# jyakaranda/A-LeGO-LOAM

Hardware: AMD Instinct MI355X
Metric: scans/sec (16x1800 LiDAR) full IP->LO->LM loop (higher is better)
Workload: dtype f32/f64

## Files before the change

### a-lego-loam_amd/csrc/alego_api.hip

```cpp
#include <hip/hip_runtime.h>

#include <cmath>
#include <cstdio>
#include <cstdlib>
#include <algorithm>
#include <cstring>
#include <mutex>
#include <string>
#include <vector>

#include "../../include/alego_mi355x.h"
#include "api_gate.h"
#include "dev_common.h"
#include "dev_mem.h"
#include "front_end.h"
#include "lm_ctx.h"
#include "lm_host.h"
#include "merge_math.h"
#include "nn_rules.h"
#include "thin_math.h"
#include "occ_math.h"
#include "loop_ctx.h"
#include "pgraph.h"
#include "prof.h"
// ... 246 lines not shown
  d.ip_scr = ip_screen_consts(d.sin_ax, d.cos_ax, d.sin_ay, d.cos_ay, d.tan_theta, d.tan_g_lo, d.tan_g_hi, d.opt_ip_screen);
  d.opt_ip_fused = env_int("ALEGO_IP_FUSED", 1) != 0;
  d.opt_ip_half = env_int("ALEGO_IP_HALF", 1) != 0;
  d.opt_cc_fused = env_int("ALEGO_CC_FUSED", 1) != 0;
  d.opt_cc_tile = env_int("ALEGO_CC_TILE", 1) != 0;
  d.opt_ip_band = env_int("ALEGO_IP_BAND", 1) != 0;
  d.opt_fe_pick1 = env_int("ALEGO_FE_PICK1", 0) != 0;
  d.opt_fe_fused = env_int("ALEGO_FE_FUSED", 1) != 0;
  d.opt_fe_cand = env_int("ALEGO_FE_CAND", 0);
  d.opt_fe_span = env_int("ALEGO_FE_SPAN", 0);
  d.opt_lo_box_lds = env_int("ALEGO_LO_BOX_LDS", 1 << 20);
  d.opt_lo_grid = env_int("ALEGO_LO_GRID", 1) != 0;
  d.opt_fo_spin = env_int("ALEGO_FE_SPIN", 0);
  d.opt_fo_pad8 = env_int("ALEGO_FE_PAD8", 0) != 0;
  d.opt_map_merge = env_int("ALEGO_MAP_MERGE", 1) != 0;
  d.opt_solve_full_eval = env_int("ALEGO_SOLVE_FULL_EVAL", 0) != 0;
  d.fcap[F_SHARP] = d.cap_sharp * d.NS; d.fcap[F_LSHARP] = d.cap_lsharp * d.NS; d.fcap[F_FLAT] = d.cap_flat * d.NS; d.fcap[F_LFLAT] = d.N;
  d.lo_qcap_surf = d.fcap[F_FLAT]; d.lo_qcap_corner = d.fcap[F_SHARP];
  d.lo_box_cap = (d.N + LO_CH - 1) / LO_CH + d.NS;
  const size_t B = n_slots, N = d.N, NS = d.NS;
  int rc = 0;
  rc |= dalloc(h, &d.in_pts, B * ring_len * d.Pcap, false);
  rc |= dalloc(h, &d.in_n, B * ring_len);
  rc |= dalloc(h, &d.owner, B * N); rc |= dalloc(h, &d.range_img, B * N); rc |= dalloc(h, &d.flag_img, B * N);
  rc |= dalloc(h, &d.parent, B * N); rc |= dalloc(h, &d.cc_size, B * N); rc |= dalloc(h, &d.cc_rows, B * N);
  rc |= dalloc(h, &d.label_img, B * N); rc |= dalloc(h, &d.cc_label, B * N);
  d.ipb_col = nullptr; d.ipb_off = nullptr;
  if (d.NS > 16 && d.NS <= 64) { rc |= dalloc(h, &d.ipb_col, B * ipb_col_n(d)); rc |= dalloc(h, &d.ipb_off, B * ipb_off_n(d)); }
  d.ipf_own = nullptr;
  if (d.NS <= 16 && d.N <= 65535 && (d.H & 1) == 0) rc |= dalloc(h, &d.ipf_own, B * (N / 2), false);
// ... 707 lines not shown
  else if (s == "ALEGO_FE_FUSED") d.opt_fe_fused = value != 0;
  else if (s == "ALEGO_FE_CAND") d.opt_fe_cand = value;
  else if (s == "ALEGO_FE_SPAN") d.opt_fe_span = value;
  else if (s == "ALEGO_LO_BOX_LDS") d.opt_lo_box_lds = value;
  else if (s == "ALEGO_LO_GRID") d.opt_lo_grid = value != 0;
  else if (s == "ALEGO_FE_SPIN") d.opt_fo_spin = value;
  else if (s == "ALEGO_SOLVE_FULL_EVAL") d.opt_solve_full_eval = value != 0;
  else if (s == "ALEGO_FE_PAD8") d.opt_fo_pad8 = value != 0;
  else if (s == "ALEGO_FE_ERR_CLEAR") {
    if (value < -1 || value >= d.n_slots) return ALEGO_ERR_ARG;
    HIP_TRY(h, hipDeviceSynchronize());
    if (value >= 0) HIP_TRY(h, hipMemset(scal_of(d, value) + SC_FE_ERR, 0, 4));
    else HIP_TRY(h, hipMemset2D(scal_of(d, 0) + SC_FE_ERR, scal_n() * sizeof(int), 0, 4, d.n_slots));
  }
  else if (s == "ALEGO_MAP_MERGE") { if (int r = lm_host_set_map_merge(h->lm, value != 0, &h->err)) return r; d.opt_map_merge = value != 0; }
  else if (s == "ALEGO_IP_FAST") d.ip_fast = h->ip_fast_capable & value;
  else if (s == "ALEGO_POKE_GUARD") { HIP_TRY(h, hipMemset(scal_of(d, d.n_slots) + value, 0xFF, 4)); }
  else if (s == "ALEGO_GV_SMALL_MAX") { WAIT_ALL(h); return lm_host_set_gv_small_max(h->lm, value); }
  else if (s == "ALEGO_LOC_CHUNK") return lm_host_set_loc_chunk(h->lm, value);
  else if (s == "ALEGO_PG_BUDGET") graph_ctx_set_budget(&h->pg, value);
  else if (s == "ALEGO_LC_BUDGET") loop_ctx_set_budget(&h->lc, value);
  else if (s == "ALEGO_RL_BUDGET") reloc_ctx_set(&h->rl, 0, value);
  else if (s == "ALEGO_RL_BRUTE") reloc_ctx_set(&h->rl, 1, value);
  else if (s == "ALEGO_SHARD_SLICE") return lm_host_debug_slice(h->lm, value & 0xff, value >> 8, &h->err);
  else { h->err = "unknown option " + s; return ALEGO_ERR_ARG; }
  return 0;
}

int alego_loop_detect(const alego_params* P, const float* keyposes6, const double* stamps, int32_t n, const double cur_xyz[3]) {
  if (!P || n <= 0 || !keyposes6 || !stamps || !cur_xyz) return -1;
// ... 834 lines not shown
```

### a-lego-loam_amd/csrc/dev_common.h

```cpp
#ifndef ALEGO_DEV_COMMON_H_
#define ALEGO_DEV_COMMON_H_

#include <hip/hip_runtime.h>
#include <stdint.h>

#include "../../include/alego_params.h"
#include "wave.h"
#include "ip_pred.h"

#define IPB_NM 9
#define IP_OWNER_TAG 0x40000000

struct DevCtx {
  alego_params P;
  int n_slots, ring_len;
  int slot0, n_launch;
  int N, H, NS;
  int Pcap;
  int cap_sharp, cap_lsharp, cap_flat;
  double sin_ax, cos_ax, sin_ay, cos_ay;
  double inv_res_x, inv_res_y;
  const double2* ip_rowtab;
  const double2* ip_coltab;
  const double* ip_colfrac;
// ... 1 lines not shown
  unsigned h_magic;
  double tan_g_lo, tan_g_hi;
  double tan_theta;
  IpScreenConsts ip_scr;
  int opt_ip_fused;
  int opt_ip_half;
  int opt_cc_fused;
  int opt_cc_tile;
  int opt_fe_pick1;
  int opt_fe_fused;
  int opt_fe_cand;
  int opt_fe_span;
  int opt_lo_box_lds;
  int opt_map_merge;
  int opt_ip_screen;
  int opt_solve_full_eval;
  float4* in_pts;
  int* in_n;
  const float4* bag_pts;
  const int* bag_n;
  const int2* bag_src;
  int n_bags, bag_len, replay_bag;
  int fs_cur, fs_last;
  int* owner;
  float* range_img;
  uint8_t* flag_img;
  int* parent;
  int* cc_size;
  unsigned long long* cc_rows;
  unsigned long long* ipb_col;
// ... 170 lines not shown
```

### a-lego-loam_amd/csrc/kernels_lm.hip

```cpp
#include <cstddef>
#include <cstring>

#include "../../include/alego_mi355x.h"
#include "dev_cost.h"
#include "nn_rules.h"
#include "remap_math.h"
#include "prof.h"
#include "kf_store.h"
#include "gmap.h"
#include "vgrid.h"

#define LM_BLOCK 256

DEV_INLINE double* ldp(const LmCtx& L, int slot) { return L.ld + (size_t)slot * LD_COUNT; }
DEV_INLINE int* lip(const LmCtx& L, int slot) { return L.li + (size_t)slot * LI_COUNT; }

DEV_INLINE void lm_map_update(const LmCtx& L, int slot, int* li, int merge) {
  const int nkf = li[LI_NKF];
  if (nkf == 0) return;
  int* rec = L.rec + (size_t)slot * L.K;
  const int cnt = li[LI_REC_CNT];
  bool changed = false;
  if (cnt < L.K) {
    const int nk = min(nkf, L.K);
    changed = li[LI_DIRTY] != 0;
// ... 101 lines not shown
  if (j == nk - 1 && blockIdx.x == 0 && threadIdx.x == 0) { li[LI_KRAW_C] = offc + nc; li[LI_KRAW_S] = offs + ns + no; }
}

__global__ void __launch_bounds__(LM_BLOCK) lm_total(DevCtx d, LmCtx L) {
  const int slot = blockIdx.y + d.slot0;
  int* li = lip(L, slot);
  if (!li[LI_RUN]) return;
  int ns = li[LI_NCUR_S], no = li[LI_NCUR_O];
  if (ns + no > L.total_cap) { no = L.total_cap - ns; if (threadIdx.x == 0 && blockIdx.x == 0) li[LI_OVERFLOW] = 1; }
  const float4* s = L.cur_surf_ds + (size_t)slot * L.kf_cap_s;
  const float4* o = L.cur_outl_ds + (size_t)slot * L.kf_cap_o;
  float4* t = L.cur_total + (size_t)slot * L.total_cap;
  for (int i = blockIdx.x * LM_BLOCK + threadIdx.x; i < ns; i += gridDim.x * LM_BLOCK) t[i] = s[i];
  for (int i = blockIdx.x * LM_BLOCK + threadIdx.x; i < no; i += gridDim.x * LM_BLOCK) t[ns + i] = o[i];
  if (blockIdx.x == 0 && threadIdx.x == 0) li[LI_NTOTAL] = ns + no;
}

DEV_INLINE int grid_cell(const GridGeom& g, float x, float y, float z, int* cx, int* cy, int* cz) {
  *cx = nn_lm_coord(x, g.inv) - g.ox; *cy = nn_lm_coord(y, g.inv) - g.oy; *cz = nn_lm_coord(z, g.inv) - g.oz;
  return nn_lm_index(*cx, *cy, *cz, g.gx, g.gy, g.gz);
}

__global__ void __launch_bounds__(LM_BLOCK) lm_grid_build(DevCtx d, LmCtx L) {
  const int slot = blockIdx.y + d.slot0, m = blockIdx.x;
  const int* li = lip(L, slot);
  if (!li[LI_REBUILD]) return;
  __shared__ GridGeom s_g;
  __shared__ int s[LM_BLOCK / 64];
  __shared__ int s_run;
  if (threadIdx.x == 0) {
// ... 921 lines not shown
void launch_lm_prepare(const DevCtx& d, const LmCtx& L, int stage, int run_hint, int par, hipStream_t st) {
  const bool small = run_hint == 0 || stage == 2;
  const dim3 grid = small ? dim3(1, 1, d.n_launch) : dim3(8, 3, d.n_launch);
  ALEGO_LAUNCH(lm_prepare, grid, dim3(small ? 64 : LM_BLOCK), 0, st, d, L, stage, run_hint, par);
}
void launch_lm_stage(const DevCtx& d, const LmCtx& L, int run_hint, int par, hipStream_t st) {
  const dim3 grid = run_hint == 0 ? dim3(1, 1, d.n_launch) : dim3(8, 3, d.n_launch);
  ALEGO_LAUNCH(lm_stage, grid, dim3(run_hint == 0 ? 64 : LM_BLOCK), 0, st, d, L, run_hint, par);
}
void launch_lm_concat(const DevCtx& d, const LmCtx& L, hipStream_t st) {
  ALEGO_LAUNCH(lm_concat, dim3(2, L.K, d.n_launch), dim3(LM_BLOCK), 0, st, d, L);
}
void launch_lm_total(const DevCtx& d, const LmCtx& L, hipStream_t st) {
  ALEGO_LAUNCH(lm_total, dim3(8, d.n_launch), dim3(LM_BLOCK), 0, st, d, L);
}
void launch_lm_grid(const DevCtx& d, const LmCtx& L, hipStream_t st) {
  ALEGO_LAUNCH(lm_grid_build, dim3(2, d.n_launch), dim3(LM_BLOCK), 0, st, d, L);
}
void launch_lm_solve(const DevCtx& d, const LmCtx& L, bool remap, hipStream_t st) {
  const size_t lds = LM_SOLVE_RED_BYTES + L.solve_row_bytes;
  if (remap) {
    if (d.opt_solve_full_eval) ALEGO_LAUNCH(lm_solve_remap_full_eval, dim3(d.n_launch), dim3(LM_SOLVE_T), lds, st, d, L);
    else ALEGO_LAUNCH(lm_solve_remap, dim3(d.n_launch), dim3(LM_SOLVE_T), lds, st, d, L);
  } else if (d.opt_solve_full_eval) {
    ALEGO_LAUNCH(lm_solve_full_eval, dim3(d.n_launch), dim3(LM_SOLVE_T), lds, st, d, L);
  } else {
    ALEGO_LAUNCH(lm_solve, dim3(d.n_launch), dim3(LM_SOLVE_T), lds, st, d, L);
  }
}
int launch_lm_register(const DevCtx& d, const LmCtx& L, hipStream_t st, int (*allreduce)(void*, double*, size_t, hipStream_t), void* ar_ctx) {
// ... 70 lines not shown
```

### a-lego-loam_amd/csrc/kernels_voxel.hip

```cpp
#include <algorithm>
#include <cstring>

#include <hip/hip_runtime.h>

#include <vector>

#include "voxel.h"
#include "wave.h"
#include "vgrid.h"
#include "dev_mem.h"
#include "prof.h"

typedef unsigned long long u64;

__device__ __forceinline__ bool vx_enabled(const VoxJob& J) { return J.enable == nullptr || *J.enable != 0; }

#ifndef VX_SMALL_MAX
#define VX_SMALL_MAX 8192
#endif

#ifndef VG_T
#define VG_T 512
#endif
#define VG_W (VG_T / 64)
#define VG_DMAX 9
#define VG_ND (1 << VG_DMAX)
#define VG_U 4

__device__ __forceinline__ int vg_div(int pos, int seglen, double inv_seglen) {
  int q = (int)((double)pos * inv_seglen);
  if (q * seglen > pos) --q;
  if ((q + 1) * seglen <= pos) ++q;
  return q;
}
// ... 385 lines not shown
    for (int j = blockIdx.x; j < nbig; j += min((int)gridDim.x, V.grid_big)) {
      vox_big_job(V, V.list_big[j], vs_smem_k);
      __syncthreads();
    }
  }
}

__global__ void __launch_bounds__(256) vox_plan(VoxCtx V) {
  __shared__ int s_n[2];
  if (threadIdx.x < 2) s_n[threadIdx.x] = 0;
  __syncthreads();
  for (int j = threadIdx.x; j < V.njobs; j += 256) {
    const VoxJob J = V.jobs[j];
    if (!vx_enabled(J)) continue;
    const int n = min(*J.n_in, J.cap);
    if (n == 0) { *J.n_out = 0; if (J.mode == 1 && J.n_sel_out) J.n_sel_out[(size_t)(J.out_sel ? *J.out_sel : 0) * J.n_sel_stride] = 0; continue; }
    if (n <= VX_SMALL_MAX) V.list_small[atomicAdd(&s_n[0], 1)] = j;
    else V.list_big[atomicAdd(&s_n[1], 1)] = j;
  }
  __syncthreads();
  if (threadIdx.x < 2) V.cnt[threadIdx.x] = s_n[threadIdx.x];
}

#define VX_SMALL_LDS (8 * VX_SMALL_MAX + 2 * VS_W * VS_ND)
int vox_create(VoxCtx* V, const VoxJob* jobs, int njobs, std::string* err) {
  std::memset(V, 0, sizeof(*V));
  if (hipFuncSetAttribute(reinterpret_cast<const void*>(vox_small), hipFuncAttributeMaxDynamicSharedMemorySize, VX_SMALL_LDS) != hipSuccess) { *err = "vox_create: hipFuncSetAttribute"; return -2; }
  std::vector<VoxJob> h(jobs, jobs + njobs);
  size_t total = 0;
  for (auto& j : h) {
    j.off = (int)total;
    if (j.cap > VX_SMALL_MAX) total += (size_t)j.cap;
  }
  if (total > 0x7fffffffull) { *err = "vox_create: scratch exceeds 2^31 elements"; return -3; }
  V->njobs = njobs; V->total = (unsigned)total;
  hipError_t e = hipSuccess;
  DevPool mem;
  auto A = [&](auto** p, size_t count) { if (e == hipSuccess) e = mem.get(p, count, true); };
  A(&V->jobs, (size_t)njobs); A(&V->bbox, (size_t)njobs * 8);
  A(&V->keys, total); A(&V->pairs_a, total); A(&V->pairs_b, total);
  A(&V->list_small, (size_t)njobs); A(&V->list_big, (size_t)njobs); A(&V->cnt, 2);
  V->grid_small = V->grid_big = njobs;
  if (e == hipSuccess) e = hipMemcpy(V->jobs, h.data(), sizeof(VoxJob) * njobs, hipMemcpyHostToDevice);
  if (e != hipSuccess) { std::memset(V, 0, sizeof(*V)); *err = std::string("vox_create: ") + hipGetErrorString(e); return -2; }
  mem.detach();
  return 0;
}

void vox_destroy(VoxCtx* V) {
  DevPool mem;
  for (void* p : {(void*)V->jobs, (void*)V->bbox, (void*)V->keys, (void*)V->pairs_a, (void*)V->pairs_b, (void*)V->list_small, (void*)V->list_big, (void*)V->cnt}) mem.adopt(p);
  std::memset(V, 0, sizeof(*V));
}

int vox_run(const VoxCtx& V, hipStream_t st, std::string* err) {
  (void)err;
  if (V.njobs == 0) return 0;
  ALEGO_LAUNCH(vox_plan, dim3(1), dim3(256), 0, st, V);
  static_assert(VG_T == VX_SB && VG_LDS_BYTES <= VX_SMALL_LDS, "large jobs run in vox_small's workgroups and LDS");
  ALEGO_LAUNCH(vox_small, dim3(std::max(V.grid_small, V.grid_big)), dim3(VX_SB), (size_t)VX_SMALL_LDS, st, V);
  return 0;
}
```

### a-lego-loam_amd/csrc/lm_ctx.h

```cpp
#ifndef ALEGO_LM_CTX_H_
#define ALEGO_LM_CTX_H_
#include "dev_common.h"
#include "lm_rows.h"

enum {
  LI_NKF = 0,
  LI_DIRTY,
  LI_RUN,
  LI_REBUILD,
  LI_FRAME,
  LI_FLAGS,
  LI_NCC, LI_NSC,
  LI_SUM0, LI_SUM1,
  LI_KF_ADDED, LI_OPTIMIZED,
  LI_KRAW_C, LI_KRAW_S, LI_KDS_C, LI_KDS_S,
  LI_NIN_C, LI_NIN_S, LI_NIN_O,
  LI_NCUR_C, LI_NCUR_S, LI_NCUR_O,
  LI_NTOTAL, LI_NTOTAL_DS,
  LI_NREBUILD,
  LI_OVERFLOW,
  LI_REC_CNT,
  LI_LATEST,
  LI_NU_C, LI_NU_S,
  LI_UVALID,
  LI_PREV_CNT,
  LI_KF_PENDING,
  LI_KF_PEND_RING,
  LI_TMPN_C, LI_TMPN_S,
  LI_REBUILD_FB,
  LI_MAP_PASS,
  LI_SORT_N,
  LI_SORT_N1,
  LI_COUNT = 48
};
enum {
  LD_PARAMS = 0,
  LD_T_M2O = 6, LD_Q_M2O = 9,
  LD_T_O2L = 13, LD_Q_O2L = 16,
  LD_T_M2L = 20, LD_Q_M2L = 23,
  LD_PARAMS_IT = 27,
  LD_COSTS = 39,
  LD_LOC_P = 44,
  LD_COUNT = 48
};

struct alego_graph_edge;
struct alego_regcov;
struct alego_remap;

struct MapWork {
  int* items;
  int* count;
  int cap;
};
struct GridGeom { int ox, oy, oz; float inv; int gx, gy, gz, ncell; };


DEV_INLINE void keypose_matrix(const float* kp, float m[3][4]) {
  const float hz = 0.5f * kp[5], hy = 0.5f * kp[4], hx = 0.5f * kp[3];
  const float qz[4] = {d_cosf(hz), 0.f, 0.f, d_sinf(hz)};
  const float qy[4] = {d_cosf(hy), 0.f, d_sinf(hy), 0.f};
  const float qx[4] = {d_cosf(hx), d_sinf(hx), 0.f, 0.f};
  float t[4], q[4];
  t[0] = qz[0] * qy[0] - qz[1] * qy[1] - qz[2] * qy[2] - qz[3] * qy[3];
  t[1] = qz[0] * qy[1] + qz[1] * qy[0] + qz[2] * qy[3] - qz[3] * qy[2];
  t[2] = qz[0] * qy[2] + qz[2] * qy[0] + qz[3] * qy[1] - qz[1] * qy[3];
  t[3] = qz[0] * qy[3] + qz[3] * qy[0] + qz[1] * qy[2] - qz[2] * qy[1];
  q[0] = t[0] * qx[0] - t[1] * qx[1] - t[2] * qx[2] - t[3] * qx[3];
  q[1] = t[0] * qx[1] + t[1] * qx[0] + t[2] * qx[3] - t[3] * qx[2];
// ... 100 lines not shown
  }
}
DEV_INLINE void lm_store_outer_empty(int* li, double* ld, int outer) {
  if (outer < 2) {
    li[LI_SUM0 + outer] = 4 << 16;
    for (int k = 0; k < 6; ++k) ld[LD_PARAMS_IT + outer * 6 + k] = ld[LD_PARAMS + k];
  }
}

size_t lm_solve_row_bytes_max(), lm_solve_row_bytes_default();
int lm_configure();
void launch_lm_prepare(const DevCtx& d, const LmCtx& L, int stage, int run_hint, int par, hipStream_t st);
void launch_lm_stage(const DevCtx& d, const LmCtx& L, int run_hint, int par, hipStream_t st);
void launch_lm_concat(const DevCtx& d, const LmCtx& L, hipStream_t st);
void launch_lm_total(const DevCtx& d, const LmCtx& L, hipStream_t st);
void launch_lm_grid(const DevCtx& d, const LmCtx& L, hipStream_t st);
void launch_lm_solve(const DevCtx& d, const LmCtx& L, bool remap, hipStream_t st);
int launch_lm_register(const DevCtx& d, const LmCtx& L, hipStream_t st, int (*allreduce)(void*, double*, size_t, hipStream_t), void* ar_ctx);
void launch_lm_retransform(const DevCtx& d, const LmCtx& L, int ring, hipStream_t st);
void launch_lm_apply_correction(const DevCtx& d, const LmCtx& L, int slot, const double* rc_dev, hipStream_t st);
void launch_lm_regcov_debug(const double* blocks, const float4* qc, int n_edge, const float4* qs, int n_plane, const double* params, double huber, const double* opt,
                            alego_regcov* rec, hipStream_t st);
void regcov_host(const double* acc28, const double* params6, int n_edge, int n_plane, const double* opt, alego_regcov* out);
void regcov_normal_host(const double* params6, const double* edge_rows9, int n_edge, const double* plane_rows7, int n_plane, double huber, double* acc28);
void remap_host(const double* acc28, const double* params6, int n_edge, int n_plane, double eig_min, alego_remap* out);
int remap_step_host(const double* H21, const double* g6, const double* scale6, double radius, const double* proj36, double* step6, double* mcc);
void launch_map_update(const DevCtx& d, const LmCtx& L, const MapWork& W, hipStream_t st);
void launch_map_accum(const DevCtx& d, const LmCtx& L, const MapWork& W, hipStream_t st);
void launch_loc_select(const DevCtx& d, const LmCtx& L, hipStream_t st);

// ... 2 lines not shown
```

### a-lego-loam_amd/csrc/lm_host.hip

```cpp
#include "lm_host.h"
#include "api_gate.h"
#include "dev_mem.h"

#include <cstddef>
#include <cstdio>
#include <cstdlib>
#include <algorithm>
#include <cstring>
#include <vector>

#include <rccl/rccl.h>

#include "kf_store.h"
#include "voxel.h"
#include "gmap.h"
#include "loc_math.h"
#include "pgraph.h"
#include "merge.h"
#include "merge_math.h"
#include "thin.h"
#include "thin_math.h"
#include "occ.h"
#include "loc_store.h"
#include "remap_math.h"

struct LmHost {
  alego_params P;
  int n_slots;
  int gsize;
  std::vector<hipStream_t> st;
  LmCtx L;
  std::vector<VoxCtx> vm, v2;
  std::vector<VoxCtx> vk;
  std::vector<MapWork> work;
  bool fallback_ok = true;
  ncclComm_t comm = nullptr;
  std::string dist_err;
  DevPool mem;
  std::vector<long> frames;
  GvCtx gv;
  int* arc_off = nullptr;
  VoxCtx vloc;
  bool vloc_made = false;
  int loc_chunk = 128;
  DevBuf<MgPair> mg_pairs;
  DevBuf<int2> mg_items;
  DevBuf<int> mg_tail;
  DevBuf<MgMove> mg_moves;
  DevBuf<ThJob> th_jobs;
// ... 111 lines not shown
  if (hipMemcpy(L.ld, ld.data(), ld.size() * sizeof(double), hipMemcpyHostToDevice) != hipSuccess) { *err = "lm_host_create: upload failed"; lm_host_destroy(lm); return nullptr; }
  std::vector<int> li0(B * LI_COUNT, 0);
  for (size_t b = 0; b < B; ++b) li0[b * LI_COUNT + LI_LATEST] = -1;
  if (hipMemcpy(L.li, li0.data(), li0.size() * sizeof(int), hipMemcpyHostToDevice) != hipSuccess) { *err = "lm_host_create: upload failed"; lm_host_destroy(lm); return nullptr; }
  for (size_t g = 0; g < st.size(); ++g) {
  std::vector<VoxJob> jm, j1, j2, jk;
  for (size_t b = g * gsize; b < B && b < (g + 1) * (size_t)gsize; ++b) {
    int* li = L.li + b * LI_COUNT;
    if (lm->fallback_ok) {
      jm.push_back(VoxJob{L.map_corner_raw + b * L.map_cap_c, li + LI_KRAW_C, L.map_corner_ds + b * L.map_cap_c, li + LI_KDS_C, li + LI_REBUILD_FB, P.lm_leaf_corner, L.map_cap_c, L.map_cap_c, li + LI_OVERFLOW, 0});
      jm.push_back(VoxJob{L.map_surf_raw + b * L.map_cap_s, li + LI_KRAW_S, L.map_surf_ds + b * L.map_cap_s, li + LI_KDS_S, li + LI_REBUILD_FB, P.lm_leaf_surf, L.map_cap_s, L.map_cap_s, li + LI_OVERFLOW, 0});
    }
    j1.push_back(VoxJob{L.in_corner + b * L.in_cap_c, li + LI_NIN_C, L.cur_corner_ds + b * L.kf_cap_c, li + LI_NCUR_C, li + LI_RUN, P.lm_leaf_corner, L.in_cap_c, L.kf_cap_c, li + LI_OVERFLOW, 0});
    j1.push_back(VoxJob{L.in_surf + b * L.in_cap_s, li + LI_NIN_S, L.cur_surf_ds + b * L.kf_cap_s, li + LI_NCUR_S, li + LI_RUN, P.lm_leaf_surf, L.in_cap_s, L.kf_cap_s, li + LI_OVERFLOW, 0});
    j1.push_back(VoxJob{L.in_outl + b * L.in_cap_o, li + LI_NIN_O, L.cur_outl_ds + b * L.kf_cap_o, li + LI_NCUR_O, li + LI_RUN, P.lm_leaf_outlier, L.in_cap_o, L.kf_cap_o, li + LI_OVERFLOW, 0});
    j2.push_back(VoxJob{L.cur_total + b * L.total_cap, li + LI_NTOTAL, L.cur_total_ds + b * L.total_cap, li + LI_NTOTAL_DS, li + LI_RUN, P.lm_leaf_surf, L.total_cap, L.total_cap, li + LI_OVERFLOW, 0});
    kf_sort_jobs(L, P, (int)b, &jk);
  }
  const int ns = (int)j1.size() / 3;
  jm.insert(jm.end(), j1.begin(), j1.end());
  jm.insert(jm.end(), jk.begin(), jk.end());
  if (vox_create(&lm->vm[g], jm.data(), (int)jm.size(), err) || vox_create(&lm->v2[g], j2.data(), (int)j2.size(), err) ||
      vox_create(&lm->vk[g], jk.data(), (int)jk.size(), err)) { lm_host_destroy(lm); return nullptr; }
  const bool big_scans = d.N > 8 * 8192;
  lm->vm[g].grid_small = 3 * ns + std::max(2, ns / 2);
  if (const char* e = getenv("ALEGO_VOX_GRID_DIV")) { const int dv = std::max(1, atoi(e)); lm->vm[g].grid_small = std::max(2, lm->vm[g].grid_small / dv); lm->v2[g].grid_small = std::max(1, lm->v2[g].grid_small / dv); }
  lm->vm[g].grid_big = (!d.opt_map_merge || big_scans) ? std::max(2, ns / 2) : std::min(8, std::max(2, ns / 2));
  lm->v2[g].grid_big = big_scans ? std::max(2, ns / 2) : std::max(1, ns / 16);
  lm->vk[g].grid_small = 2; lm->vk[g].grid_big = 2;
  MapWork& W = lm->work[g];
  W.cap = std::max(4096, 64 * ns);
  if (!A(lm, &W.items, (size_t)W.cap, err) || !A(lm, &W.count, 2, err)) { lm_host_destroy(lm); return nullptr; }
  }
  return lm;
}

void lm_host_destroy(LmHost* lm) {
  if (!lm) return;
  if (lm->comm) { (void)ncclCommDestroy(lm->comm); lm->comm = nullptr; }
  for (auto& v : lm->vm) vox_destroy(&v);
  for (auto& v : lm->v2) vox_destroy(&v);
  for (auto& v : lm->vk) vox_destroy(&v);
  if (lm->vloc_made) vox_destroy(&lm->vloc);
  gv_destroy(&lm->gv);
// ... 7 lines not shown
  static const bool on = getenv("ALEGO_DEBUG_SYNC") != nullptr;
  if (!on) return true;
  hipError_t e = hipStreamSynchronize(st);
  if (e == hipSuccess) e = hipGetLastError();
  fprintf(stderr, "[alego dbg] %s: %s\n", what, hipGetErrorString(e));
  if (e != hipSuccess) { *err = std::string(what) + ": " + hipGetErrorString(e); return false; }
  return true;
}

static int map_sequence(LmHost* lm, const DevCtx& d, const LmCtx& L, int g, hipStream_t st, std::string* err) {
  if (!d.opt_map_merge) {
    if (!lm->fallback_ok) { *err = "ALEGO_MAP_MERGE=0 needs the handle to be created with it (more than 64 slots)"; return ALEGO_ERR_ARG; }
    launch_lm_concat(d, L, st);
    if (!dbg_sync(st, "lm_concat", err)) return ALEGO_ERR_HIP;
  }
  if (int r = vox_run(lm->vm[g], st, err)) return r;
  if (!dbg_sync(st, "vox round 1", err)) return ALEGO_ERR_HIP;
  launch_map_update(d, L, lm->work[g], st);
  if (!dbg_sync(st, "map_update", err)) return ALEGO_ERR_HIP;
  if (d.opt_map_merge) {
    launch_map_accum(d, L, lm->work[g], st);
    if (!dbg_sync(st, "map_accum", err)) return ALEGO_ERR_HIP;
  }
  launch_lm_grid(d, L, st);
  if (!dbg_sync(st, "lm_grid", err)) return ALEGO_ERR_HIP;
  return 0;
}

static int lm_allreduce(void* ctx, double* buf, size_t count, hipStream_t st) {
  LmHost* lm = static_cast<LmHost*>(ctx);
  const ncclResult_t r = ncclAllReduce(buf, buf, count, ncclDouble, ncclSum, lm->comm, st);
// ... 20 lines not shown
    par = (int)(A->k & 1);
    if (A->k >= 2 && hipStreamWaitEvent(A->front, A->back_same, 0) != hipSuccess) { *err = "hipStreamWaitEvent failed"; return ALEGO_ERR_HIP; }
    if (hint != 0 && A->k >= 1 && hipStreamWaitEvent(A->front, A->back_other, 0) != hipSuccess) { *err = "hipStreamWaitEvent failed"; return ALEGO_ERR_HIP; }
    launch_lm_stage(d, L, hint, par, A->front);
    if (hipEventRecord(A->staged, A->front) != hipSuccess || hipStreamWaitEvent(st, A->staged, 0) != hipSuccess) { *err = "event hand-over to the LaserMapping stream failed"; return ALEGO_ERR_HIP; }
    stage = 2;
  }
  launch_lm_prepare(d, L, stage, hint, par, st);
  if (!dbg_sync(st, "lm_prepare", err)) return ALEGO_ERR_HIP;
  if (n_run == 0) return 0;
  if (L.loc_on) {
    launch_loc_select(d, L, st);
    if (!dbg_sync(st, "loc_select", err)) return ALEGO_ERR_HIP;
  }
  if (int r = map_sequence(lm, d, L, g, st, err)) return r;
  launch_lm_total(d, L, st);
  if (int r = vox_run(lm->v2[g], st, err)) return r;
  if (!dbg_sync(st, "vox total", err)) return ALEGO_ERR_HIP;
  if (int r = launch_lm_register(d, L, st, lm->comm ? &lm_allreduce : nullptr, lm)) { *err = "sharded registration: " + lm->dist_err; return r; }
  if (!dbg_sync(st, "lm_register", err)) return ALEGO_ERR_HIP;
  return 0;
}

static void clear_run_flags_outside(LmHost* lm, const DevCtx& d) {
  const int g = d.slot0 / lm->gsize;
  const int lo = g * lm->gsize, hi = std::min(lm->n_slots, lo + lm->gsize);
  if (d.slot0 == lo && d.slot0 + d.n_launch == hi) return;
  for (int s = lo; s < hi; ++s) {
    if (s >= d.slot0 && s < d.slot0 + d.n_launch) continue;
    (void)hipMemsetAsync(lm->L.li + (size_t)s * LI_COUNT + LI_RUN, 0, sizeof(int), lm->st[g]);
  }
}
// ... 1136 lines not shown
```

### a-lego-loam_amd/csrc/vgrid.h

```cpp
#ifndef ALEGO_VGRID_H_
#define ALEGO_VGRID_H_
#include <hip/hip_runtime.h>

__device__ __forceinline__ unsigned vgr_enc(float f) {
  const unsigned b = (unsigned)__float_as_int(f);
  return b ^ ((b >> 31) ? 0xFFFFFFFFu : 0x80000000u);
}
__device__ __forceinline__ float vgr_dec(unsigned u) { return __int_as_float((int)((u >> 31) ? (u ^ 0x80000000u) : ~u)); }
__device__ __forceinline__ void vgr_box_load(const unsigned* bb, float mn[3], float mx[3]) {
#pragma unroll
  for (int a = 0; a < 3; ++a) { mn[a] = vgr_dec(bb[a]); mx[a] = vgr_dec(~bb[4 + a]); }
}

__device__ __forceinline__ void vgr_box_add(float mn[3], float mx[3], float4 p) {
  mn[0] = fminf(mn[0], p.x); mn[1] = fminf(mn[1], p.y); mn[2] = fminf(mn[2], p.z);
  mx[0] = fmaxf(mx[0], p.x); mx[1] = fmaxf(mx[1], p.y); mx[2] = fmaxf(mx[2], p.z);
}

__device__ __forceinline__ bool vgr_leaf_too_small(const float mn[3], const float mx[3], float inv) {
  const long long dx = (long long)((mx[0] - mn[0]) * inv) + 1, dy = (long long)((mx[1] - mn[1]) * inv) + 1, dz = (long long)((mx[2] - mn[2]) * inv) + 1;
  return dx * dy * dz > 2147483647LL;
}

struct VgrGeom {
  int minb[3], divb[3];
  unsigned mul1, mul2;
  unsigned long long T;
};
__device__ __forceinline__ VgrGeom vgr_geom(const float mn[3], const float mx[3], float inv) {
  VgrGeom g;
#pragma unroll
  for (int a = 0; a < 3; ++a) { g.minb[a] = (int)floorf(mn[a] * inv); g.divb[a] = (int)floorf(mx[a] * inv) - g.minb[a] + 1; }
  g.mul1 = (unsigned)g.divb[0];
  g.mul2 = (unsigned)g.divb[0] * (unsigned)g.divb[1];
  g.T = (unsigned long long)(unsigned)g.divb[0] * (unsigned)g.divb[1] * (unsigned)g.divb[2];
  return g;
}
__device__ __forceinline__ int vgr_bits(unsigned long long T) {
  if (T > 0xFFFFFFFFull || T == 0) return 32;
  return T > 1 ? 32 - __clz((int)(unsigned)(T - 1)) : 0;
}
__device__ __forceinline__ void vgr_coords(const VgrGeom& g, float4 p, float inv, int* i0, int* i1, int* i2) {
  *i0 = (int)(floorf(p.x * inv) - (float)g.minb[0]);
  *i1 = (int)(floorf(p.y * inv) - (float)g.minb[1]);
  *i2 = (int)(floorf(p.z * inv) - (float)g.minb[2]);
}
__device__ __forceinline__ unsigned vgr_id(const VgrGeom& g, float4 p, float inv) {
  int i0, i1, i2;
  vgr_coords(g, p, inv, &i0, &i1, &i2);
  return (unsigned)i0 + (unsigned)i1 * g.mul1 + (unsigned)i2 * g.mul2;
}

#define VKEY_B (1 << 20)
__device__ __forceinline__ bool vkey_holds_box(const float mn[3], const float mx[3], float inv) {
#pragma unroll
  for (int a = 0; a < 3; ++a)
    if (floorf(mn[a] * inv) < -(float)VKEY_B || floorf(mx[a] * inv) > (float)(VKEY_B - 1)) return false;
  return true;
}
__device__ __forceinline__ unsigned long long vkey_pack(int ix, int iy, int iz) {
  const int B = VKEY_B;
  const unsigned long long x = (unsigned long long)(unsigned)min(max(ix + B, 0), 2 * B - 1), y = (unsigned long long)(unsigned)min(max(iy + B, 0), 2 * B - 1),
                           z = (unsigned long long)(unsigned)min(max(iz + B, 0), 2 * B - 1);
  return (z << 42) | (y << 21) | x;
}
__device__ __forceinline__ unsigned long long vkey_of(const float4& p, float inv) {
  return vkey_pack((int)floorf(p.x * inv), (int)floorf(p.y * inv), (int)floorf(p.z * inv));
}

#endif
```

### a-lego-loam_amd/csrc/voxel.h

```cpp
#ifndef ALEGO_VOXEL_H_
#define ALEGO_VOXEL_H_
#include <hip/hip_runtime.h>

#include <string>

struct VoxJob {
  const float4* in;
  const int* n_in;
  float4* out;
  int* n_out;
  const int* enable;
  float leaf;
  int cap;
  int out_cap;
  int* overflow;
  int off;
  int mode;
  const int* out_sel;
  int out_stride;
  float* box_out;
  int* n_sel_out;
  int n_sel_stride;
};

struct VoxCtx {
  VoxJob* jobs;
  int njobs;
  unsigned* bbox;
  unsigned* keys;
  unsigned long long *pairs_a, *pairs_b;
  int *list_small, *list_big, *cnt;
  int grid_small, grid_big;
  unsigned total;
};

int vox_create(VoxCtx* V, const VoxJob* jobs, int njobs, std::string* err);
void vox_destroy(VoxCtx* V);
int vox_run(const VoxCtx& V, hipStream_t st, std::string* err);

#endif
```

Measured before the change: 490,900.

## Fuse outlier voxelization and surf/outlier total merge into one LM kernel

Adds a single-block-per-slot kernel that voxel-downsamples small outlier clouds in LDS and then merges the already-sorted surface voxels with the outlier voxels into the total downsampled cloud. Only slots whose merge cannot be proven sound fall back to the generic voxel path, through a device-built work list. This removes the separate outlier voxel job, the concat kernel and most of the generic total voxel pass. The cost is an O(n^2) rank sort in LDS, a dependence on the surface cloud being key-sorted (checked at runtime, with fallback), and extra code paths behind a default-on flag.

After: 498,600 (median of 6 runs). 1.6% higher.

```diff
diff --git a/a-lego-loam_amd/csrc/alego_api.hip b/a-lego-loam_amd/csrc/alego_api.hip
--- a/a-lego-loam_amd/csrc/alego_api.hip
+++ b/a-lego-loam_amd/csrc/alego_api.hip
@@ -284,6 +284,7 @@
   d.opt_fo_spin = env_int("ALEGO_FE_SPIN", 0);
   d.opt_fo_pad8 = env_int("ALEGO_FE_PAD8", 0) != 0;
   d.opt_map_merge = env_int("ALEGO_MAP_MERGE", 1) != 0;
+  d.opt_lm_total_merge = env_int("ALEGO_LM_TOTAL_MERGE", 1) != 0;
   d.opt_solve_full_eval = env_int("ALEGO_SOLVE_FULL_EVAL", 0) != 0;
   d.fcap[F_SHARP] = d.cap_sharp * d.NS; d.fcap[F_LSHARP] = d.cap_lsharp * d.NS; d.fcap[F_FLAT] = d.cap_flat * d.NS; d.fcap[F_LFLAT] = d.N;
   d.lo_qcap_surf = d.fcap[F_FLAT]; d.lo_qcap_corner = d.fcap[F_SHARP];
@@ -1021,6 +1022,7 @@
     else HIP_TRY(h, hipMemset2D(scal_of(d, 0) + SC_FE_ERR, scal_n() * sizeof(int), 0, 4, d.n_slots));
   }
   else if (s == "ALEGO_MAP_MERGE") { if (int r = lm_host_set_map_merge(h->lm, value != 0, &h->err)) return r; d.opt_map_merge = value != 0; }
+  else if (s == "ALEGO_LM_TOTAL_MERGE") d.opt_lm_total_merge = value != 0;
   else if (s == "ALEGO_IP_FAST") d.ip_fast = h->ip_fast_capable & value;
   else if (s == "ALEGO_POKE_GUARD") { HIP_TRY(h, hipMemset(scal_of(d, d.n_slots) + value, 0xFF, 4)); }
   else if (s == "ALEGO_GV_SMALL_MAX") { WAIT_ALL(h); return lm_host_set_gv_small_max(h->lm, value); }
diff --git a/a-lego-loam_amd/csrc/dev_common.h b/a-lego-loam_amd/csrc/dev_common.h
--- a/a-lego-loam_amd/csrc/dev_common.h
+++ b/a-lego-loam_amd/csrc/dev_common.h
@@ -39,6 +39,7 @@
   int opt_lo_box_lds;
   int opt_map_merge;
   int opt_ip_screen;
+  int opt_lm_total_merge;
   int opt_solve_full_eval;
   float4* in_pts;
   int* in_n;
diff --git a/a-lego-loam_amd/csrc/kernels_lm.hip b/a-lego-loam_amd/csrc/kernels_lm.hip
--- a/a-lego-loam_amd/csrc/kernels_lm.hip
+++ b/a-lego-loam_amd/csrc/kernels_lm.hip
@@ -9,6 +9,7 @@
 #include "kf_store.h"
 #include "gmap.h"
 #include "vgrid.h"
+#include "vox_merge.h"
 
 #define LM_BLOCK 256
 
@@ -140,6 +141,188 @@
   for (int i = blockIdx.x * LM_BLOCK + threadIdx.x; i < ns; i += gridDim.x * LM_BLOCK) t[i] = s[i];
   for (int i = blockIdx.x * LM_BLOCK + threadIdx.x; i < no; i += gridDim.x * LM_BLOCK) t[ns + i] = o[i];
   if (blockIdx.x == 0 && threadIdx.x == 0) li[LI_NTOTAL] = ns + no;
+}
+
+#define LT_T 256
+#define LT_B 8
+DEV_INLINE void lt_box_reduce(float mn[3], float mx[3], float (*s_red)[LT_T / 64]) {
+  const int lane = threadIdx.x & 63, wave = threadIdx.x >> 6;
+  __syncthreads();
+#pragma unroll
+  for (int a = 0; a < 3; ++a) {
+    bfly_minmax_f32(mn[a], mx[a]);
+    if (lane == 0) { s_red[a][wave] = mn[a]; s_red[3 + a][wave] = mx[a]; }
+  }
+  __syncthreads();
+#pragma unroll
+  for (int a = 0; a < 3; ++a) {
+    mn[a] = s_red[a][0]; mx[a] = s_red[3 + a][0];
+#pragma unroll
+    for (int w = 1; w < LT_T / 64; ++w) { mn[a] = fminf(mn[a], s_red[a][w]); mx[a] = fmaxf(mx[a], s_red[3 + a][w]); }
+  }
+}
+DEV_INLINE void lt_order(const vm_u64* s_key, vm_u64* s_skey, unsigned short* s_idx, int n) {
+  __syncthreads();
+  for (int i = threadIdx.x; i < n; i += LT_T) { const int r = vm_rank(s_key, n, i); s_skey[r] = s_key[i]; s_idx[r] = (unsigned short)i; }
+  __syncthreads();
+}
+
+__global__ void __launch_bounds__(LT_T) lm_total_merge(DevCtx d, LmCtx L, LtLists W) {
+  const int slot = blockIdx.x + d.slot0, tid = threadIdx.x;
+  int* li = lip(L, slot);
+  __shared__ vm_u64 s_key[LT_OCAP], s_skey[LT_OCAP];
+  __shared__ unsigned short s_idx[LT_OCAP];
+  __shared__ int s_osb[LT_OCAP];
+  __shared__ int s_oop[LT_OCAP + 1];
+  __shared__ int s_base[LT_T];
+  __shared__ float s_red[6][LT_T / 64];
+  __shared__ int s_w[LT_T / 64];
+  int state = 0;
+  if (li[LI_RUN]) {
+    const float FMAX = 3.402823466e+38f;
+    int no = li[LI_NCUR_O];
+    const int nin = min(li[LI_NIN_O], L.in_cap_o);
+    if (nin <= LT_OCAP) {
+      const float4* in = L.in_outl + (size_t)slot * L.in_cap_o;
+      float4* out = L.cur_outl_ds + (size_t)slot * L.kf_cap_o;
+      const int cap = L.kf_cap_o;
+      const float inv = 1.0f / d.P.lm_leaf_outlier;
+      int nvox = 0, full = nin;
+      if (nin > 0) {
+        float mn[3] = {FMAX, FMAX, FMAX}, mx[3] = {-FMAX, -FMAX, -FMAX};
+        for (int i = tid; i < nin; i += LT_T) vgr_box_add(mn, mx, in[i]);
+        lt_box_reduce(mn, mx, s_red);
+        if (vgr_leaf_too_small(mn, mx, inv)) {
+          for (int i = tid; i < min(nin, cap); i += LT_T) out[i] = in[i];
+        } else {
+          const VgrGeom g = vgr_geom(mn, mx, inv);
+          for (int i = tid; i < nin; i += LT_T) s_key[i] = vgr_id(g, in[i], inv);
+          lt_order(s_key, s_skey, s_idx, nin);
+          for (int t0 = 0; t0 < nin; t0 += LT_T) {
+            const int m = t0 + tid;
+            const bool head = m < nin && (m == 0 || s_skey[m] != s_skey[m - 1]);
+            int tot;
+            const int r = nvox + block_excl_scan<LT_T / 64>(head ? 1 : 0, s_w, &tot);
+            if (head && r < cap) {
+              int b = m + 1;
+              while (b < nin && s_skey[b] == s_skey[m]) ++b;
+              out[r] = vm_centroid([&](int j) { return in[s_idx[j]]; }, m, b);
+            }
+            nvox += tot;
+          }
+          full = nvox;
+        }
+      }
+      no = min(full, cap);
+      if (tid == 0) { li[LI_NCUR_O] = no; if (full > cap) li[LI_OVERFLOW] = 1; }
+      __syncthreads();
+    }
+    const int ns = li[LI_NCUR_S];
+    if (ns + no > L.total_cap) { no = L.total_cap - ns; if (tid == 0) li[LI_OVERFLOW] = 1; }
+    const int n = ns + no, cap = L.total_cap;
+    const float4* S = L.cur_surf_ds + (size_t)slot * L.kf_cap_s;
+    const float4* O = L.cur_outl_ds + (size_t)slot * L.kf_cap_o;
+    float4* out = L.cur_total_ds + (size_t)slot * L.total_cap;
+    const float inv = 1.0f / d.P.lm_leaf_surf;
+    const int c = (ns + LT_T - 1) / LT_T, c0 = min(ns, tid * c), c1 = min(ns, c0 + c);
+    bool refuse = no > LT_OCAP;
+    int heads = 0;
+    if (!refuse && n > 0) {
+      float mn[3] = {FMAX, FMAX, FMAX}, mx[3] = {-FMAX, -FMAX, -FMAX};
+      int good = 1;
+      for (int j = tid; j < no; j += LT_T) { const float4 p = O[j]; vgr_box_add(mn, mx, p); good &= vm_finite(p); s_key[j] = vkey_of(p, inv); s_osb[j] = -1; }
+      lt_order(s_key, s_skey, s_idx, no);
+      vm_u64 kprev = 0;
+      int ole_prev = 0;
+      if (c0 > 0 && c0 < c1) { kprev = vkey_of(S[c0 - 1], inv); ole_prev = vm_count_le(s_skey, no, kprev); }
+      for (int b0 = c0; b0 < c1; b0 += LT_B) {
+        float4 p[LT_B];
+#pragma unroll
+        for (int k = 0; k < LT_B; ++k) p[k] = S[min(b0 + k, c1 - 1)];
+#pragma unroll
+        for (int k = 0; k < LT_B; ++k) {
+          const int i = b0 + k;
+          if (i < c1) {
+            vgr_box_add(mn, mx, p[k]);
+            const vm_u64 key = vkey_of(p[k], inv);
+            good &= vm_finite(p[k]) && (i == 0 || kprev <= key);
+            const int ol = vm_count_less(s_skey, no, key);
+            for (int j = ole_prev; j < ol; ++j) s_osb[j] = tid << 16 | heads;
+            heads += (i == 0 || kprev != key) ? 1 : 0;
+            kprev = key; ole_prev = vm_count_le(s_skey, no, key);
+          }
+        }
+      }
+      if ((c0 < c1 && c1 == ns) || (ns == 0 && tid == 0)) for (int j = ole_prev; j < no; ++j) s_osb[j] = tid << 16 | heads;
+      lt_box_reduce(mn, mx, s_red);
+      good = __syncthreads_and(good);
+      refuse = vm_refuse(good != 0, no, mn, mx, inv);
+    }
+    if (!refuse) {
+      int nsh;
+      const int base = block_excl_scan<LT_T / 64>(heads, s_w, &nsh);
+      s_base[tid] = base;
+      int noo = 0;
+      for (int t0 = 0; t0 < no; t0 += LT_T) {
+        const int j = t0 + tid;
+        const bool oh = j < no && s_osb[j] >= 0 && (j == 0 || s_skey[j - 1] != s_skey[j]);
+        int tot;
+        const int e = noo + block_excl_scan<LT_T / 64>(oh ? 1 : 0, s_w, &tot);
+        if (j < no) s_oop[j] = e;
+        noo += tot;
+      }
+      if (tid == 0) s_oop[no] = noo;
+      __syncthreads();
+      vm_u64 kprev = c0 > 0 && c0 < c1 ? vkey_of(S[c0 - 1], inv) : 0;
+      int hl = 0;
+      for (int b0 = c0; b0 < c1; b0 += LT_B) {
+        float4 p[LT_B + 1];
+#pragma unroll
+        for (int k = 0; k <= LT_B; ++k) p[k] = S[min(b0 + k, ns - 1)];
+#pragma unroll
+        for (int k = 0; k < LT_B; ++k) {
+          const int i = b0 + k;
+          if (i < c1) {
+            const vm_u64 key = vkey_of(p[k], inv);
+            if (i == 0 || kprev != key) {
+              const int ol = vm_count_less(s_skey, no, key), ole = vm_count_le(s_skey, no, key);
+              const int r = base + hl + s_oop[ol];
+              ++hl;
+              if (r < cap) {
+                int nsr = 1;
+                if (i + 1 < ns && vkey_of(p[k + 1], inv) == key) while (i + nsr < ns && vkey_of(S[i + nsr], inv) == key) ++nsr;
+                out[r] = vm_centroid([&](int q) { return q == 0 ? p[k] : (q < nsr ? S[i + q] : O[s_idx[ol + q - nsr]]); }, 0, nsr + ole - ol);
+              }
+            }
+            kprev = key;
+          }
+        }
+      }
+      for (int j = tid; j < no; j += LT_T) {
+        if (s_osb[j] >= 0 && (j == 0 || s_skey[j - 1] != s_skey[j])) {
+          const int r = s_base[s_osb[j] >> 16] + (s_osb[j] & 0xFFFF) + s_oop[j];
+          if (r < cap) {
+            int e = j + 1;
+            while (e < no && s_skey[e] == s_skey[j]) ++e;
+            out[r] = vm_centroid([&](int q) { return O[s_idx[q]]; }, j, e);
+          }
+        }
+      }
+      const int nvox = nsh + noo;
+      if (tid == 0) { li[LI_NTOTAL] = n; li[LI_NTOTAL_DS] = min(nvox, cap); if (nvox > cap) li[LI_OVERFLOW] = 1; li[LI_TM_FAST] += 1; }
+    } else {
+      float4* t = L.cur_total + (size_t)slot * L.total_cap;
+      for (int i = tid; i < ns; i += LT_T) t[i] = S[i];
+      for (int i = tid; i < no; i += LT_T) t[ns + i] = O[i];
+      if (tid == 0) { li[LI_NTOTAL] = n; li[LI_TM_LIST] += 1; }
+      state = n > W.small_max ? 2 : 1;
+    }
+  }
+  if (tid == 0) {
+    if (state == 1) W.list_small[atomicAdd(&W.cnt[0], 1)] = slot - L.vox_slot0;
+    else if (state == 2) W.list_big[atomicAdd(&W.cnt[1], 1)] = slot - L.vox_slot0;
+    if (blockIdx.x == 0) { W.cnt_next[0] = 0; W.cnt_next[1] = 0; }
+  }
 }
 
 DEV_INLINE int grid_cell(const GridGeom& g, float x, float y, float z, int* cx, int* cy, int* cz) {
@@ -1091,6 +1274,9 @@
 void launch_lm_total(const DevCtx& d, const LmCtx& L, hipStream_t st) {
   ALEGO_LAUNCH(lm_total, dim3(8, d.n_launch), dim3(LM_BLOCK), 0, st, d, L);
 }
+void launch_lm_total_merge(const DevCtx& d, const LmCtx& L, const LtLists& W, hipStream_t st) {
+  ALEGO_LAUNCH(lm_total_merge, dim3(d.n_launch), dim3(LT_T), 0, st, d, L, W);
+}
 void launch_lm_grid(const DevCtx& d, const LmCtx& L, hipStream_t st) {
   ALEGO_LAUNCH(lm_grid_build, dim3(2, d.n_launch), dim3(LM_BLOCK), 0, st, d, L);
 }
diff --git a/a-lego-loam_amd/csrc/kernels_voxel.hip b/a-lego-loam_amd/csrc/kernels_voxel.hip
--- a/a-lego-loam_amd/csrc/kernels_voxel.hip
+++ b/a-lego-loam_amd/csrc/kernels_voxel.hip
@@ -14,10 +14,6 @@
 typedef unsigned long long u64;
 
 __device__ __forceinline__ bool vx_enabled(const VoxJob& J) { return J.enable == nullptr || *J.enable != 0; }
-
-#ifndef VX_SMALL_MAX
-#define VX_SMALL_MAX 8192
-#endif
 
 #ifndef VG_T
 #define VG_T 512
@@ -433,6 +429,7 @@
     const VoxJob J = V.jobs[j];
     if (!vx_enabled(J)) continue;
     const int n = min(*J.n_in, J.cap);
+    if (V.skip_on && J.skip_le > 0 && n <= J.skip_le) continue;
     if (n == 0) { *J.n_out = 0; if (J.mode == 1 && J.n_sel_out) J.n_sel_out[(size_t)(J.out_sel ? *J.out_sel : 0) * J.n_sel_stride] = 0; continue; }
     if (n <= VX_SMALL_MAX) V.list_small[atomicAdd(&s_n[0], 1)] = j;
     else V.list_big[atomicAdd(&s_n[1], 1)] = j;
@@ -458,7 +455,7 @@
   auto A = [&](auto** p, size_t count) { if (e == hipSuccess) e = mem.get(p, count, true); };
   A(&V->jobs, (size_t)njobs); A(&V->bbox, (size_t)njobs * 8);
   A(&V->keys, total); A(&V->pairs_a, total); A(&V->pairs_b, total);
-  A(&V->list_small, (size_t)njobs); A(&V->list_big, (size_t)njobs); A(&V->cnt, 2);
+  A(&V->list_small, (size_t)njobs); A(&V->list_big, (size_t)njobs); A(&V->cnt, 6);
   V->grid_small = V->grid_big = njobs;
   if (e == hipSuccess) e = hipMemcpy(V->jobs, h.data(), sizeof(VoxJob) * njobs, hipMemcpyHostToDevice);
   if (e != hipSuccess) { std::memset(V, 0, sizeof(*V)); *err = std::string("vox_create: ") + hipGetErrorString(e); return -2; }
@@ -480,3 +477,10 @@
   ALEGO_LAUNCH(vox_small, dim3(std::max(V.grid_small, V.grid_big)), dim3(VX_SB), (size_t)VX_SMALL_LDS, st, V);
   return 0;
 }
+
+int vox_run_listed(const VoxCtx& V, hipStream_t st, std::string* err) {
+  (void)err;
+  if (V.njobs == 0) return 0;
+  ALEGO_LAUNCH(vox_small, dim3(std::max(V.grid_small, V.grid_big)), dim3(VX_SB), (size_t)VX_SMALL_LDS, st, V);
+  return 0;
+}
diff --git a/a-lego-loam_amd/csrc/lm_ctx.h b/a-lego-loam_amd/csrc/lm_ctx.h
--- a/a-lego-loam_amd/csrc/lm_ctx.h
+++ b/a-lego-loam_amd/csrc/lm_ctx.h
@@ -31,6 +31,8 @@
   LI_MAP_PASS,
   LI_SORT_N,
   LI_SORT_N1,
+  LI_TM_FAST,
+  LI_TM_LIST,
   LI_COUNT = 48
 };
 enum {
@@ -53,6 +55,7 @@
   int* count;
   int cap;
 };
+struct LtLists { int *list_small, *list_big, *cnt, *cnt_next; int small_max; };
 struct GridGeom { int ox, oy, oz; float inv; int gx, gy, gz, ncell; };
 
 
@@ -183,6 +186,7 @@
 void launch_lm_stage(const DevCtx& d, const LmCtx& L, int run_hint, int par, hipStream_t st);
 void launch_lm_concat(const DevCtx& d, const LmCtx& L, hipStream_t st);
 void launch_lm_total(const DevCtx& d, const LmCtx& L, hipStream_t st);
+void launch_lm_total_merge(const DevCtx& d, const LmCtx& L, const LtLists& W, hipStream_t st);
 void launch_lm_grid(const DevCtx& d, const LmCtx& L, hipStream_t st);
 void launch_lm_solve(const DevCtx& d, const LmCtx& L, bool remap, hipStream_t st);
 int launch_lm_register(const DevCtx& d, const LmCtx& L, hipStream_t st, int (*allreduce)(void*, double*, size_t, hipStream_t), void* ar_ctx);
diff --git a/a-lego-loam_amd/csrc/lm_host.hip b/a-lego-loam_amd/csrc/lm_host.hip
--- a/a-lego-loam_amd/csrc/lm_host.hip
+++ b/a-lego-loam_amd/csrc/lm_host.hip
@@ -13,6 +13,7 @@
 
 #include "kf_store.h"
 #include "voxel.h"
+#include "vox_merge.h"
 #include "gmap.h"
 #include "loc_math.h"
 #include "pgraph.h"
@@ -33,6 +34,7 @@
   std::vector<VoxCtx> vm, v2;
   std::vector<VoxCtx> vk;
   std::vector<MapWork> work;
+  std::vector<int> tm_grid1, tm_grid, tm_par;
   bool fallback_ok = true;
   ncclComm_t comm = nullptr;
   std::string dist_err;
@@ -174,6 +176,7 @@
     j1.push_back(VoxJob{L.in_corner + b * L.in_cap_c, li + LI_NIN_C, L.cur_corner_ds + b * L.kf_cap_c, li + LI_NCUR_C, li + LI_RUN, P.lm_leaf_corner, L.in_cap_c, L.kf_cap_c, li + LI_OVERFLOW, 0});
     j1.push_back(VoxJob{L.in_surf + b * L.in_cap_s, li + LI_NIN_S, L.cur_surf_ds + b * L.kf_cap_s, li + LI_NCUR_S, li + LI_RUN, P.lm_leaf_surf, L.in_cap_s, L.kf_cap_s, li + LI_OVERFLOW, 0});
     j1.push_back(VoxJob{L.in_outl + b * L.in_cap_o, li + LI_NIN_O, L.cur_outl_ds + b * L.kf_cap_o, li + LI_NCUR_O, li + LI_RUN, P.lm_leaf_outlier, L.in_cap_o, L.kf_cap_o, li + LI_OVERFLOW, 0});
+    j1.back().skip_le = LT_OCAP;
     j2.push_back(VoxJob{L.cur_total + b * L.total_cap, li + LI_NTOTAL, L.cur_total_ds + b * L.total_cap, li + LI_NTOTAL_DS, li + LI_RUN, P.lm_leaf_surf, L.total_cap, L.total_cap, li + LI_OVERFLOW, 0});
     kf_sort_jobs(L, P, (int)b, &jk);
   }
@@ -184,10 +187,17 @@
       vox_create(&lm->vk[g], jk.data(), (int)jk.size(), err)) { lm_host_destroy(lm); return nullptr; }
   const bool big_scans = d.N > 8 * 8192;
   lm->vm[g].grid_small = 3 * ns + std::max(2, ns / 2);
-  if (const char* e = getenv("ALEGO_VOX_GRID_DIV")) { const int dv = std::max(1, atoi(e)); lm->vm[g].grid_small = std::max(2, lm->vm[g].grid_small / dv); lm->v2[g].grid_small = std::max(1, lm->v2[g].grid_small / dv); }
+  int tm_grid1 = 2 * ns + std::max(2, ns / 2);
+  if (const char* e = getenv("ALEGO_VOX_GRID_DIV")) {
+    const int dv = std::max(1, atoi(e));
+    lm->vm[g].grid_small = std::max(2, lm->vm[g].grid_small / dv); lm->v2[g].grid_small = std::max(1, lm->v2[g].grid_small / dv);
+    tm_grid1 = std::max(2, tm_grid1 / dv);
+  }
   lm->vm[g].grid_big = (!d.opt_map_merge || big_scans) ? std::max(2, ns / 2) : std::min(8, std::max(2, ns / 2));
   lm->v2[g].grid_big = big_scans ? std::max(2, ns / 2) : std::max(1, ns / 16);
   lm->vk[g].grid_small = 2; lm->vk[g].grid_big = 2;
+  lm->tm_grid1.push_back(tm_grid1); lm->tm_par.push_back(0);
+  lm->tm_grid.push_back(std::max(1, ns / 16));
   MapWork& W = lm->work[g];
   W.cap = std::max(4096, 64 * ns);
   if (!A(lm, &W.items, (size_t)W.cap, err) || !A(lm, &W.count, 2, err)) { lm_host_destroy(lm); return nullptr; }
@@ -225,7 +235,9 @@
     launch_lm_concat(d, L, st);
     if (!dbg_sync(st, "lm_concat", err)) return ALEGO_ERR_HIP;
   }
-  if (int r = vox_run(lm->vm[g], st, err)) return r;
+  VoxCtx V1 = lm->vm[g];
+  if (d.opt_lm_total_merge) { V1.skip_on = 1; V1.grid_small = lm->tm_grid1[g]; }
+  if (int r = vox_run(V1, st, err)) return r;
   if (!dbg_sync(st, "vox round 1", err)) return ALEGO_ERR_HIP;
   launch_map_update(d, L, lm->work[g], st);
   if (!dbg_sync(st, "map_update", err)) return ALEGO_ERR_HIP;
@@ -276,8 +288,20 @@
     if (!dbg_sync(st, "loc_select", err)) return ALEGO_ERR_HIP;
   }
   if (int r = map_sequence(lm, d, L, g, st, err)) return r;
-  launch_lm_total(d, L, st);
-  if (int r = vox_run(lm->v2[g], st, err)) return r;
+  if (d.opt_lm_total_merge) {
+    VoxCtx V2 = lm->v2[g];
+    int* const cnt = V2.cnt;
+    const int par = lm->tm_par[g];
+    lm->tm_par[g] ^= 1;
+    V2.cnt = cnt + 2 + 2 * par;
+    launch_lm_total_merge(d, L, LtLists{V2.list_small, V2.list_big, V2.cnt, cnt + 2 + 2 * (par ^ 1), VX_SMALL_MAX}, st);
+    if (!dbg_sync(st, "lm_total_merge", err)) return ALEGO_ERR_HIP;
+    V2.grid_small = V2.grid_big = lm->tm_grid[g];
+    if (int r = vox_run_listed(V2, st, err)) return r;
+  } else {
+    launch_lm_total(d, L, st);
+    if (int r = vox_run(lm->v2[g], st, err)) return r;
+  }
   if (!dbg_sync(st, "vox total", err)) return ALEGO_ERR_HIP;
   if (int r = launch_lm_register(d, L, st, lm->comm ? &lm_allreduce : nullptr, lm)) { *err = "sharded registration: " + lm->dist_err; return r; }
   if (!dbg_sync(st, "lm_register", err)) return ALEGO_ERR_HIP;
diff --git a/a-lego-loam_amd/csrc/vgrid.h b/a-lego-loam_amd/csrc/vgrid.h
--- a/a-lego-loam_amd/csrc/vgrid.h
+++ b/a-lego-loam_amd/csrc/vgrid.h
@@ -1,7 +1,15 @@
 #ifndef ALEGO_VGRID_H_
 #define ALEGO_VGRID_H_
+#if defined(__HIPCC__)
 #include <hip/hip_runtime.h>
+#define VGR_FN __host__ __device__ __forceinline__
+#else
+#include <math.h>
+struct float4 { float x, y, z, w; };
+#define VGR_FN static inline
+#endif
 
+#if defined(__HIPCC__)
 __device__ __forceinline__ unsigned vgr_enc(float f) {
   const unsigned b = (unsigned)__float_as_int(f);
   return b ^ ((b >> 31) ? 0xFFFFFFFFu : 0x80000000u);
@@ -12,12 +20,14 @@
   for (int a = 0; a < 3; ++a) { mn[a] = vgr_dec(bb[a]); mx[a] = vgr_dec(~bb[4 + a]); }
 }
 
-__device__ __forceinline__ void vgr_box_add(float mn[3], float mx[3], float4 p) {
+#endif
+
+VGR_FN void vgr_box_add(float mn[3], float mx[3], float4 p) {
   mn[0] = fminf(mn[0], p.x); mn[1] = fminf(mn[1], p.y); mn[2] = fminf(mn[2], p.z);
   mx[0] = fmaxf(mx[0], p.x); mx[1] = fmaxf(mx[1], p.y); mx[2] = fmaxf(mx[2], p.z);
 }
 
-__device__ __forceinline__ bool vgr_leaf_too_small(const float mn[3], const float mx[3], float inv) {
+VGR_FN bool vgr_leaf_too_small(const float mn[3], const float mx[3], float inv) {
   const long long dx = (long long)((mx[0] - mn[0]) * inv) + 1, dy = (long long)((mx[1] - mn[1]) * inv) + 1, dz = (long long)((mx[2] - mn[2]) * inv) + 1;
   return dx * dy * dz > 2147483647LL;
 }
@@ -27,7 +37,7 @@
   unsigned mul1, mul2;
   unsigned long long T;
 };
-__device__ __forceinline__ VgrGeom vgr_geom(const float mn[3], const float mx[3], float inv) {
+VGR_FN VgrGeom vgr_geom(const float mn[3], const float mx[3], float inv) {
   VgrGeom g;
 #pragma unroll
   for (int a = 0; a < 3; ++a) { g.minb[a] = (int)floorf(mn[a] * inv); g.divb[a] = (int)floorf(mx[a] * inv) - g.minb[a] + 1; }
@@ -36,35 +46,38 @@
   g.T = (unsigned long long)(unsigned)g.divb[0] * (unsigned)g.divb[1] * (unsigned)g.divb[2];
   return g;
 }
+#if defined(__HIPCC__)
 __device__ __forceinline__ int vgr_bits(unsigned long long T) {
   if (T > 0xFFFFFFFFull || T == 0) return 32;
   return T > 1 ? 32 - __clz((int)(unsigned)(T - 1)) : 0;
 }
-__device__ __forceinline__ void vgr_coords(const VgrGeom& g, float4 p, float inv, int* i0, int* i1, int* i2) {
+#endif
+VGR_FN void vgr_coords(const VgrGeom& g, float4 p, float inv, int* i0, int* i1, int* i2) {
   *i0 = (int)(floorf(p.x * inv) - (float)g.minb[0]);
   *i1 = (int)(floorf(p.y * inv) - (float)g.minb[1]);
   *i2 = (int)(floorf(p.z * inv) - (float)g.minb[2]);
 }
-__device__ __forceinline__ unsigned vgr_id(const VgrGeom& g, float4 p, float inv) {
+VGR_FN unsigned vgr_id(const VgrGeom& g, float4 p, float inv) {
   int i0, i1, i2;
   vgr_coords(g, p, inv, &i0, &i1, &i2);
   return (unsigned)i0 + (unsigned)i1 * g.mul1 + (unsigned)i2 * g.mul2;
 }
 
 #define VKEY_B (1 << 20)
-__device__ __forceinline__ bool vkey_holds_box(const float mn[3], const float mx[3], float inv) {
+VGR_FN bool vkey_holds_box(const float mn[3], const float mx[3], float inv) {
 #pragma unroll
   for (int a = 0; a < 3; ++a)
     if (floorf(mn[a] * inv) < -(float)VKEY_B || floorf(mx[a] * inv) > (float)(VKEY_B - 1)) return false;
   return true;
 }
-__device__ __forceinline__ unsigned long long vkey_pack(int ix, int iy, int iz) {
+VGR_FN int vkey_clamp(int v, int hi) { return v < 0 ? 0 : (v > hi ? hi : v); }
+VGR_FN unsigned long long vkey_pack(int ix, int iy, int iz) {
   const int B = VKEY_B;
-  const unsigned long long x = (unsigned long long)(unsigned)min(max(ix + B, 0), 2 * B - 1), y = (unsigned long long)(unsigned)min(max(iy + B, 0), 2 * B - 1),
-                           z = (unsigned long long)(unsigned)min(max(iz + B, 0), 2 * B - 1);
+  const unsigned long long x = (unsigned long long)(unsigned)vkey_clamp(ix + B, 2 * B - 1), y = (unsigned long long)(unsigned)vkey_clamp(iy + B, 2 * B - 1),
+                           z = (unsigned long long)(unsigned)vkey_clamp(iz + B, 2 * B - 1);
   return (z << 42) | (y << 21) | x;
 }
-__device__ __forceinline__ unsigned long long vkey_of(const float4& p, float inv) {
+VGR_FN unsigned long long vkey_of(const float4& p, float inv) {
   return vkey_pack((int)floorf(p.x * inv), (int)floorf(p.y * inv), (int)floorf(p.z * inv));
 }
 
diff --git a/a-lego-loam_amd/csrc/vox_merge.h b/a-lego-loam_amd/csrc/vox_merge.h
--- /dev/null
+++ b/a-lego-loam_amd/csrc/vox_merge.h
@@ -0,0 +1,45 @@
+#ifndef ALEGO_VOX_MERGE_H_
+#define ALEGO_VOX_MERGE_H_
+#include "vgrid.h"
+
+#define LT_OCAP 512
+
+typedef unsigned long long vm_u64;
+
+VGR_FN bool vm_finite(const float4& p) { return fabsf(p.x) <= 3.402823466e+38f && fabsf(p.y) <= 3.402823466e+38f && fabsf(p.z) <= 3.402823466e+38f; }
+
+VGR_FN int vm_rank(const vm_u64* key, int n, int i) {
+  const vm_u64 k = key[i];
+  int r = 0;
+  for (int j = 0; j < n; ++j) r += (key[j] < k || (key[j] == k && j < i)) ? 1 : 0;
+  return r;
+}
+
+VGR_FN int vm_count_less(const vm_u64* sorted, int n, vm_u64 key) {
+  int lo = 0, hi = n;
+  while (lo < hi) { const int mid = (lo + hi) >> 1; if (sorted[mid] < key) lo = mid + 1; else hi = mid; }
+  return lo;
+}
+VGR_FN int vm_count_le(const vm_u64* sorted, int n, vm_u64 key) {
+  int lo = 0, hi = n;
+  while (lo < hi) { const int mid = (lo + hi) >> 1; if (sorted[mid] <= key) lo = mid + 1; else hi = mid; }
+  return lo;
+}
+
+VGR_FN bool vm_refuse(bool sound, int no, const float mn[3], const float mx[3], float inv) {
+  if (!sound || no > LT_OCAP) return true;
+  if (!vkey_holds_box(mn, mx, inv) || vgr_leaf_too_small(mn, mx, inv)) return true;
+  return vgr_geom(mn, mx, inv).T > 0xFFFFFFFFull;
+}
+
+template <class At>
+VGR_FN float4 vm_centroid(At at, int a, int b) {
+  float sx = 0.f, sy = 0.f, sz = 0.f, si = 0.f;
+  for (int j = a; j < b; ++j) { const float4 p = at(j); sx += p.x; sy += p.y; sz += p.z; si += p.w; }
+  const float fn = (float)(b - a);
+  float4 c;
+  c.x = sx / fn; c.y = sy / fn; c.z = sz / fn; c.w = si / fn;
+  return c;
+}
+
+#endif
diff --git a/a-lego-loam_amd/csrc/voxel.h b/a-lego-loam_amd/csrc/voxel.h
--- a/a-lego-loam_amd/csrc/voxel.h
+++ b/a-lego-loam_amd/csrc/voxel.h
@@ -3,6 +3,10 @@
 #include <hip/hip_runtime.h>
 
 #include <string>
+
+#ifndef VX_SMALL_MAX
+#define VX_SMALL_MAX 8192
+#endif
 
 struct VoxJob {
   const float4* in;
@@ -21,6 +25,7 @@
   float* box_out;
   int* n_sel_out;
   int n_sel_stride;
+  int skip_le;
 };
 
 struct VoxCtx {
@@ -32,10 +37,12 @@
   int *list_small, *list_big, *cnt;
   int grid_small, grid_big;
   unsigned total;
+  int skip_on;
 };
 
 int vox_create(VoxCtx* V, const VoxJob* jobs, int njobs, std::string* err);
 void vox_destroy(VoxCtx* V);
 int vox_run(const VoxCtx& V, hipStream_t st, std::string* err);
+int vox_run_listed(const VoxCtx& V, hipStream_t st, std::string* err);
 
 #endif
```
